# initc3/HoneyBadgerMPC

Hardware: AMD Instinct MI355X
Metric: shares reconstructed/sec (batch open, n=64 t=21) (higher is better)
Workload: dtype u256 (integer mod p): exact int8 x int8 -> int32 byte-split GEMM on the matrix cores; the high half of every sum folded mod p on the matrix cores too, one-word Barrett quotient

## Files before the change

### honeybadgermpc_amd/csrc/hb_common.hpp

```cpp
#pragma once
#include <hip/hip_runtime.h>
#include <stdint.h>
#include <stdio.h>
#include <string.h>

#include <functional>
#include <map>
#include <mutex>
#include <string>
#include <vector>

#include "../../include/hbmpc_hip.h"
#include "fp29.hpp"

namespace hb {
struct FastMatrix;
struct Mm8Matrix;
struct Mm8wMatrix;
}
namespace hb {

struct Wide { static constexpr int NL = 9, NW = 8; };
struct Narrow { static constexpr int NL = 3, NW = 2; };

// ... 14 lines not shown
        load_digits<NL, NW>(cd, poly + (size_t)l * NW);
        mont_mul(m, cd, pw, P);
        fp_add(acc, acc, m, P);
    }
#pragma unroll
    for (int q = 0; q < NL; q++) red[tid][q] = acc[q];
    __syncthreads();
    for (int w = 64; w >= 1; w >>= 1) {
        if (tid < w) {
            uint32_t a[NL], b[NL], t[NL];
#pragma unroll
            for (int q = 0; q < NL; q++) { a[q] = red[tid][q]; b[q] = red[tid + w][q]; }
            fp_add(t, a, b, P);
#pragma unroll
            for (int q = 0; q < NL; q++) red[tid][q] = t[q];
        }
        __syncthreads();
    }
#pragma unroll
    for (int q = 0; q < NL; q++) r[q] = red[0][q];
}

__host__ __device__ inline size_t m_index(int i, int l, int n_in, int nl, int q) {
    return (((size_t)((i / OT) * n_in + l) * (size_t)nl + (size_t)q) * OT) + (size_t)(i % OT);
}
inline int m_tiles(int n_out) { return (n_out + OT - 1) / OT; }

}

struct hb_matrix {
    hb_ctx *ctx;
    int n_out, n_in;
    uint32_t *dev;
    size_t words;
    bool cached;
    int refs;
    hb::Mm8wMatrix *wide;
    bool wide_tried;
};

namespace hb {
struct TlsError {
    static std::string &slot() { static thread_local std::string s; return s; }
    TlsError &operator=(const std::string &m) { slot() = m; return *this; }
    TlsError &operator=(const char *m) { slot() = m ? m : ""; return *this; }
    const char *c_str() const { return slot().c_str(); }
    void clear() { slot().clear(); }
    bool empty() const { return slot().empty(); }
};
struct PrescaleParams {
    uint32_t pbar[9];
    uint32_t pneg[8];
    uint32_t m0, m1;
};
}
namespace hb {
enum EnvHook {
    ENV_CACHE_CAP,
    ENV_GAO_PAIR,
    ENV_MM8W_FLAT,
    ENV_MM8W_RQ,
    ENV_MM8W_TILE16,
    ENV_MM8_NO_SKIP,
    ENV_NO_EVAL_FEW,
    ENV_NO_FUSED_SMALL,
    ENV_NO_FUSED_VALIDATE,
    ENV_NO_MFMA,
    ENV_NO_MFMA_DECODE,
    ENV_NO_MFMA_WIDE,
    ENV_NO_NARROW_FAST,
    ENV_NO_QUICK,
    ENV_NO_QUICK_PLAN,
    ENV_NTT_STAGE_LOOP,
    ENV_PROBE_WGS,
    ENV_QUICK_NO_CAND,
    ENV_UPLOAD_MODE,
    ENV_WB_NO_GAO,
    ENV_WB_NO_UNIFORM,
    ENV_COUNT
};
const char *env_hook(EnvHook h);
void env_reload();
}
struct hb_ctx {
    int device;
    int n_limbs;
    hb::FpParams<9> pw;
    hb::FpParams<3> pn;
    uint64_t p_limbs[4];
    std::recursive_mutex mu;
    int api_depth = 0;
    hb::TlsError err;
    std::map<std::string, hb_matrix *> mcache;
    std::map<std::vector<int32_t>, int32_t *> icache;
    std::map<std::string, void *> dcache;
    std::map<std::string, hb::FastMatrix *> fcache;
    std::map<std::string, hb::Mm8Matrix *> m8cache;
    struct CacheSlot { uint64_t tick; bool pinned; std::function<void()> drop; };
    std::map<std::string, CacheSlot> lru;
    uint64_t lru_clock = 0;
    size_t cache_cap = 192;
    int32_t *flag_dev;
    hb::PrescaleParams psc;
    int psc_state = 0;
    std::map<std::string, void *> ptcache;
    struct QuickSlot { void *buf = nullptr; size_t cap = 0; void *ev = nullptr; };
// ... 234 lines not shown
```

### honeybadgermpc_amd/csrc/hb_mfma.hip

```cpp
#include <atomic>

#include "hb_mm8.hpp"

namespace hb {

#include "hb_mm8_body.inc"

#ifdef HB_MM8_TIMING
__device__ unsigned long long g_mm8_t[2048 * 8];
#define MM8_T(k) do { const unsigned long long tn_ = __builtin_amdgcn_s_memtime(); tacc[k] += tn_ - tlast; tlast = tn_; } while (0)
#else
#define MM8_T(k) do { } while (0)
#endif
template <int NKB, bool CHECK, bool RAGGED, bool SKIP>
__global__ __launch_bounds__(256, 2) void k_mm8(const int4 *__restrict__ a8, const uint32_t *__restrict__ crowd,
                                                const uint32_t *__restrict__ zero_src,
                                                const uint32_t *__restrict__ in_pk, int64_t in_sc, int64_t in_sl,
                                                const int32_t *__restrict__ in_rows, int64_t in_count, int d,
                                                uint32_t *__restrict__ out_pk, int64_t out_sc, int64_t out_sl, int64_t out_count,
                                                const int32_t *__restrict__ check_mask, const int32_t *__restrict__ check_rows, int32_t *__restrict__ mismatch,
                                                uint32_t *__restrict__ copy_dst, int64_t copy_sc, int64_t copy_sl, int64_t copy_count, int copy_rows,
                                                int n_out, int n_rt, int tpw, int64_t n_chunks, int64_t n_units, BarrettParams bp) {
    extern __shared__ uint4 mm8_lds[];
    const int lane = threadIdx.x & 63, wave = __builtin_amdgcn_readfirstlane(threadIdx.x >> 6);
// ... 311 lines not shown
    uint64_t cy = 0;
    for (size_t i = 0; i < a.size(); i++) {
        uint64_t t = (uint64_t)a[i] + (i < b.size() ? b[i] : 0) + cy;
        a[i] = (uint32_t)t; cy = t >> 32;
    }
}
Big big_divmod(const Big &x, const Big &p, Big *q) {
    Big r(p.size() + 1, 0), pp(p); pp.push_back(0);
    if (q) q->assign(x.size(), 0);
    for (int bit = (int)x.size() * 32 - 1; bit >= 0; bit--) {
        uint32_t in = (x[bit >> 5] >> (bit & 31)) & 1u;
        for (size_t i = r.size(); i-- > 0;) r[i] = (r[i] << 1) | (i ? r[i - 1] >> 31 : in);
        if (big_ge(r, pp)) { big_sub(r, pp); if (q) (*q)[bit >> 5] |= 1u << (bit & 31); }
    }
    r.pop_back();
    return r;
}
Big big_shl(const Big &a, int bits, size_t words) {
    Big r(words, 0);
    for (size_t i = 0; i < a.size(); i++) {
        const size_t w = i + bits / 32; const int s = bits % 32;
        if (w < words) r[w] |= a[i] << s;
        if (s && w + 1 < words) r[w + 1] |= a[i] >> (32 - s);
    }
    return r;
}

}

namespace hb {

bool prescale_params(hb_ctx *ctx) {
    if (ctx->psc_state) return ctx->psc_state > 0;
    ctx->psc_state = -1;
    if (ctx->n_limbs != 4 || (ctx->p_limbs[3] >> 62) == 0) return false;
    Big p(8);
    for (int i = 0; i < 4; i++) { p[2 * i] = (uint32_t)ctx->p_limbs[i]; p[2 * i + 1] = (uint32_t)(ctx->p_limbs[i] >> 32); }
    Big pw9(p); pw9.push_back(0);
    Big pb(9, 0); pb[8] = 1u << 5;
    big_sub(pb, pw9);
    for (int k = 0; k < 9; k++) {
        const int bit = 29 * k, j = bit >> 5, sft = bit & 31;
        const uint64_t v = pb[j] | ((uint64_t)(j + 1 < 9 ? pb[j + 1] : 0) << 32);
        ctx->psc.pbar[k] = (uint32_t)(v >> sft) & DMASK;
    }
    Big pn(9, 0); pn[8] = 1;
    big_sub(pn, pw9);
    for (int k = 0; k < 8; k++) ctx->psc.pneg[k] = pn[k];
    Big two290(10, 0); two290[9] = 1u << 2;
    Big mu; big_divmod(two290, p, &mu);
    const uint64_t muv = mu[0] | ((uint64_t)mu[1] << 32);
    ctx->psc.m0 = (uint32_t)muv & DMASK;
    ctx->psc.m1 = (uint32_t)(muv >> LB);
    ctx->psc_state = 1;
    return true;
}

void mm8_free(Mm8Matrix *m) {
    if (!m) return;
    (void)hipFree(m->a8); (void)hipFree(m->crow); (void)hipFree(m->zero);
    delete m;
}

int mm8_shared(hb_ctx *ctx, const Mm8Shared **out, hipStream_t s) {
    if (ctx->mm8_shared) { *out = static_cast<const Mm8Shared *>(ctx->mm8_shared); return HB_OK; }
    if (ctx->n_limbs != 4 || (ctx->p_limbs[3] >> 62) == 0 || !prescale_params(ctx)) return fail(ctx, HB_ERR_UNSUPPORTED, "mm8: modulus");
    Mm8Shared *sh = new Mm8Shared();
    memset(sh, 0, sizeof *sh);
    Big p(8);
    for (int k = 0; k < 4; k++) { p[2 * k] = (uint32_t)ctx->p_limbs[k]; p[2 * k + 1] = (uint32_t)(ctx->p_limbs[k] >> 32); }
    uint32_t shift8[8];
    if (!fold_tables(ctx, 16, sh->fold_host, sh->bp.c384, &sh->bp.mu, shift8)) { delete sh; return fail(ctx, HB_ERR_UNSUPPORTED, "mm8: fold table"); }
    {
        Big pn(9, 0); pn[8] = 1;
        Big pw9(p); pw9.push_back(0);
        big_sub(pn, pw9);
        for (int k = 0; k < 8; k++) sh->bp.pneg[k] = pn[k];
    }
    auto digits9 = [](const Big &v, uint32_t *dg) {
        for (int k = 0; k < 9; k++) {
            const int bit = 29 * k, j = bit >> 5, sft = bit & 31;
            const uint64_t w = (uint64_t)(j < (int)v.size() ? v[j] : 0) | ((uint64_t)(j + 1 < (int)v.size() ? v[j + 1] : 0) << 32);
            dg[k] = (uint32_t)(w >> sft) & DMASK;
        }
    };
    Big biasmod;
    { Big bt(14, 0); for (int c = 0; c < MM8_NC; c++) { Big t(1, (uint32_t)MM8_BIAS); big_add(bt, big_shl(t, 8 * c, 14)); } biasmod = big_divmod(bt, p, nullptr); }
    { Big sft(shift8, shift8 + 8); if (!big_ge(biasmod, sft)) big_add(biasmod, p); big_sub(biasmod, sft); }
    digits9(biasmod, sh->biasmod);
    {
        Big c80(8, 0x80808080u);
        Big r261(9, 0); r261[8] = 1u << 5;
        digits9(big_divmod(big_mul(c80, r261), p, nullptr), sh->c80r);
    }
    if (hipMalloc(&sh->fold_dev, sizeof sh->fold_host) != hipSuccess) { delete sh; return fail(ctx, HB_ERR_HIP, "mm8: hipMalloc(fold table)"); }
    if (int rc = upload_table(ctx, sh->fold_dev, sh->fold_host, sizeof sh->fold_host, s)) { (void)hipFree(sh->fold_dev); delete sh; return rc; }
    ctx->mm8_shared = sh;
    *out = sh;
    return HB_OK;
}

void mm8_shared_free(hb_ctx *ctx) {
    Mm8Shared *sh = static_cast<Mm8Shared *>(ctx->mm8_shared);
    if (!sh) return;
    (void)hipFree(sh->fold_dev);
    delete sh;
// ... 171 lines not shown
```

### honeybadgermpc_amd/csrc/hb_mfma_fused.hip

```cpp
#include <math.h>

#include <algorithm>
#include <atomic>

#include "hb_mm8.hpp"

namespace hb {

#include "hb_mm8_body.inc"

constexpr int FS_WAVES = 8, FS_TPW = 4;
#ifdef HB_MM8_TIMING
__device__ unsigned long long g_fs_t[256 * 8 * 8];
#define FS_T(k) do { const unsigned long long tn_ = __builtin_amdgcn_s_memtime(); tacc[k] += tn_ - tlast; tlast = tn_; } while (0)
#else
#define FS_T(k) do { } while (0)
#endif
constexpr int FS_MAXD = 24, FS_MAXC = 104;
constexpr size_t FS_LDS_LIMIT = 156 * 1024;

struct FsIdx { uint16_t z[FS_MAXD], xz[FS_MAXD], zc[FS_MAXC], xzc[FS_MAXC]; };
struct FsPick { const uint4 *cand; const uint32_t *cand_crow; int n_coef, nc; uint16_t zc[FS_MAXC]; };
struct FsSplit { uint32_t terms[FS_WAVES]; };
constexpr int FS_CAND_MAXN = 128;

__host__ __device__ inline size_t fs_lds_bytes(int n_rt, int nkb) {
    return ((size_t)n_rt * 64 + (size_t)n_rt * nkb * 2 * 64 + (size_t)2 * FS_TPW * nkb * 4 * 64 + MM8_FOLD_Q) * 16 + (size_t)(32 + 16 * n_rt) * 4;
}

template <int NKB>
__global__ __launch_bounds__(64 * FS_WAVES, 2) void k_mm8f(const int4 *__restrict__ a8, const uint32_t *__restrict__ crowd, const v4i *__restrict__ foldg,
                                                          const uint32_t *__restrict__ KT, const PrescaleParams PP,
                                                          const uint32_t *__restrict__ in_pk, int64_t in_sc, int64_t in_sl, const int32_t *__restrict__ in_rows,
                                                          int64_t in_count, int d, const int32_t *__restrict__ rowmode,
                                                          uint32_t *__restrict__ out_pk, int64_t out_sc, int64_t out_sl, int64_t out_count,
                                                          int32_t *__restrict__ mismatch, int32_t *__restrict__ first_bad, uint32_t *__restrict__ bad_map,
                                                          int n_out, int n_rt, int64_t n_chunks, int64_t n_units, BarrettParams bp, const FsDone done, const FsPick pick,
                                                          const FsSplit split) {
    constexpr int NT = 64 * FS_WAVES, NL = 9, NW = 8;
    extern __shared__ uint4 fs_lds[];
    const int lane = threadIdx.x & 63, wave = __builtin_amdgcn_readfirstlane(threadIdx.x >> 6);
    const int n = lane & 15, g = lane >> 4;
    uint32_t *crl = reinterpret_cast<uint32_t *>(fs_lds);
    int4 *abuf = reinterpret_cast<int4 *>(fs_lds + n_rt * 64);
    uint4 *xbuf = fs_lds + n_rt * 64 + n_rt * NKB * 2 * 64;
    constexpr int bufsz = FS_TPW * NKB * 4 * 64;
    int32_t *rowl = reinterpret_cast<int32_t *>(xbuf + 2 * bufsz);
    int32_t *maskl = rowl + 32;
    v4i *foldl = reinterpret_cast<v4i *>(maskl + 16 * n_rt);

    if (threadIdx.x < 32) {
        const int lc = (int)threadIdx.x < d ? (int)threadIdx.x : d - 1;
        rowl[threadIdx.x] = in_rows ? in_rows[lc] : lc;
    }
    uint4 pk_piece = make_uint4(0, 0, 0, 0), pk_crow = make_uint4(0, 0, 0, 0);
    const int pk_e = threadIdx.x;
    const bool pk_has_piece = pick.cand && pk_e < pick.nc * NKB * 8, pk_has_crow = pick.cand && pk_e < pick.nc * 4;
    if (pk_has_piece) {
        const int j = pk_e / (NKB * 8), pc = pk_e - j * (NKB * 8);
        pk_piece = pick.cand[(size_t)pick.zc[j] * (NKB * 8) + pc];
    }
    if (pk_has_crow) pk_crow = reinterpret_cast<const uint4 *>(pick.cand_crow)[(size_t)pick.zc[pk_e >> 2] * 4 + (pk_e & 3)];
    for (int i = threadIdx.x; i < n_rt * 16; i += NT) maskl[i] = i < n_out ? rowmode[i] : 0;
    for (int i = threadIdx.x; i < n_rt * 64; i += NT) fs_lds[i] = reinterpret_cast<const uint4 *>(crowd)[i];
    for (int i = threadIdx.x; i < n_rt * NKB * 2 * 64; i += NT) abuf[i] = a8[i];
    for (int i = threadIdx.x; i < 2 * bufsz; i += NT) xbuf[i] = make_uint4(0, 0, 0, 0);
    if (threadIdx.x < MM8_FOLD_Q) foldl[threadIdx.x] = foldg[threadIdx.x];
    if (pick.cand) {
        __syncthreads();
        auto put = [&](int e, const uint4 &v) {
            const int j = e / (NKB * 8), pc = e - j * (NKB * 8);
            const int ri = pick.n_coef + j, rt = ri >> 4, r16 = ri & 15, r = 4 * (r16 & 3) + (r16 >> 2);
            const int kb = pc >> 3, grp = (pc >> 2) & 1, gg = pc & 3;
            reinterpret_cast<uint4 *>(abuf)[((rt * NKB + kb) * 2 + grp) * 64 + r + 16 * gg] = v;
        };
        if (pk_has_piece) put(pk_e, pk_piece);
        for (int e = pk_e + NT; e < pick.nc * NKB * 8; e += NT) {
            const int j = e / (NKB * 8), pc = e - j * (NKB * 8);
            put(e, pick.cand[(size_t)pick.zc[j] * (NKB * 8) + pc]);
        }
        if (pk_has_crow) fs_lds[(pick.n_coef + (pk_e >> 2)) * 4 + (pk_e & 3)] = pk_crow;
        for (int j = threadIdx.x; j < pick.nc; j += NT) maskl[pick.n_coef + j] = (int32_t)pick.zc[j] + 1;
    }
    __syncthreads();

    const int n_pairs = FS_TPW * n_rt;
    const uint32_t my_terms = (uint32_t)__builtin_amdgcn_readfirstlane((int)split.terms[wave]);

    auto scale_unit = [&](int64_t unit, uint4 *dst, uint32_t terms) {
        int64_t chunk = unit * 64 + lane;
        if (chunk >= n_chunks) chunk = n_chunks - 1;
        const int t = lane >> 4;
        uint32_t xw[NW];
        bool ok = false;
        auto fetch = [&](int l, uint32_t (&w)[NW], bool &okk) {
            const int64_t idx = chunk * in_sc + (int64_t)rowl[l] * in_sl;
            okk = idx < in_count;
            load_words<NW>(w, in_pk + (okk ? idx : 0) * NW);
        };
        terms &= d < 32 ? (1u << d) - 1u : ~0u;
        int l = terms ? __builtin_ctz(terms) : d;
        if (l < d) fetch(l, xw, ok);
        while (l < d) {
            terms &= terms - 1u;
            const int ln = terms ? __builtin_ctz(terms) : d;
            uint32_t xn[NW];
            bool okn = false;
            if (ln < d) fetch(ln, xn, okn);
            else {
#pragma unroll
                for (int k = 0; k < NW; k++) xn[k] = 0;
            }
            const uint32_t *__restrict__ T = KT + (size_t)l * (NL * NL);
            uint32_t xd[NL];
            unpack<NL, NW>(xd, xw);
            uint64_t col[NL + 1];
#pragma unroll
            for (int j = 0; j <= NL; j++) col[j] = 0;
#pragma unroll
            for (int q = 0; q < NL; q++)
#pragma unroll
                for (int j = 0; j < NL; j++) col[j] += (uint64_t)xd[q] * T[q * NL + j];
            uint32_t v[NL + 1];
#pragma unroll
            for (int k = 0; k < NL; k++) { v[k] = (uint32_t)col[k] & DMASK; col[k + 1] += col[k] >> LB; }
            v[NL] = (uint32_t)col[NL];
            const uint64_t mid = (uint64_t)v[9] * PP.m0 + (uint64_t)v[8] * PP.m1 + (((uint64_t)v[8] * PP.m0) >> LB);
            const uint64_t qh = (uint64_t)v[9] * PP.m1 + (mid >> LB);
            const uint32_t q0 = (uint32_t)qh & DMASK, q1 = (uint32_t)(qh >> LB);
            uint64_t dc[NL];
#pragma unroll
            for (int k = 0; k < NL; k++) {
                dc[k] = v[k] + (uint64_t)q0 * PP.pbar[k];
                if (k > 0) dc[k] += (uint64_t)q1 * PP.pbar[k - 1];
            }
            uint32_t r[NL];
#pragma unroll
            for (int k = 0; k < NL; k++) {
                r[k] = (uint32_t)dc[k] & DMASK;
                if (k < NL - 1) dc[k + 1] += dc[k] >> LB;
            }
            uint32_t w[NW];
            pack<NL, NW>(w, r);
            if (PP.pneg[NW - 1] >> 31) {
#pragma unroll
                for (int k = 0; k < NW; k++) w[k] = ok ? w[k] : 0u;
            } else {
                uint32_t u[NW];
                unsigned cy = 0;
#pragma unroll
                for (int k = 0; k < NW; k++) u[k] = __builtin_addc(w[k], PP.pneg[k], cy, &cy);
                const bool take = cy || (r[NL - 1] >> 24);
#pragma unroll
                for (int k = 0; k < NW; k++) w[k] = ok ? (take ? u[k] : w[k]) : 0u;
            }
            const int kb = l >> 3, gg = (l & 7) >> 1, e = l & 1;
            uint4 *slot = dst + (size_t)(((t * NKB + kb) * 2 + e) * 2) * 64 + (n + 16 * gg);
            slot[0] = make_uint4(w[0], w[1], w[2], w[3]);
            slot[64] = make_uint4(w[4], w[5], w[6], w[7]);
#pragma unroll
            for (int k = 0; k < NW; k++) xw[k] = xn[k];
            ok = okn;
            l = ln;
        }
    };

    const v4i biasv = v4i{MM8_BIAS, MM8_BIAS, MM8_BIAS, MM8_BIAS};
    uint32_t k256 = 256u, k16m = 1u << 24;
    int32_t s1 = 1, s256 = 256, s64k = 1 << 16, s16m = 1 << 24;
    uint32_t u1 = 1u;
    asm volatile("" : "+s"(k256), "+s"(k16m), "+s"(s1), "+s"(s256), "+s"(s64k), "+s"(s16m), "+s"(u1));
    const v4i *fold_lane = reinterpret_cast<const v4i *>(reinterpret_cast<const char *>(foldl) + (g == (n >> 2) ? 16 * n : 256));

    int buf = 0;
    int64_t unit = blockIdx.x;
#ifdef HB_MM8_TIMING
    unsigned long long tacc[8] = {0, 0, 0, 0, 0, 0, 0, 0}, tlast = __builtin_amdgcn_s_memtime();
#endif
    if (unit < n_units) scale_unit(unit, xbuf, 0x01010101u << wave);
    FS_T(0);
    for (; unit < n_units; unit += gridDim.x, buf ^= 1) {
        asm volatile("s_waitcnt lgkmcnt(0)" ::: "memory");
        FS_T(7);
        __builtin_amdgcn_s_barrier();
        FS_T(1);
        if (my_terms && unit + gridDim.x < n_units) scale_unit(unit + gridDim.x, xbuf + (size_t)(buf ^ 1) * bufsz, my_terms);
        FS_T(2);
        for (int pidx = wave; pidx < n_pairs; pidx += FS_WAVES) {
            const int tl = n_rt == 2 ? (pidx >> 1) : pidx / n_rt;
            const int rt = n_rt == 2 ? ((pidx ^ (pidx >> 2)) & 1) : pidx - tl * n_rt;
            const int64_t chunk = (unit * FS_TPW + tl) * 16 + n;
            const uint4 *xs = xbuf + (size_t)buf * bufsz + (size_t)tl * NKB * 4 * 64 + lane;
            const int4 *as = abuf + (size_t)rt * NKB * 2 * 64 + lane;
            uint32_t eap[4][11], c0p[4];
            const int rows_here = n_out - 16 * rt < 16 ? n_out - 16 * rt : 16;
            const int nreg = (rows_here + 3) >> 2;
            const uint32_t xs_addr = (uint32_t)(uintptr_t)(__attribute__((address_space(3))) const void *)xs;
            const uint32_t as_addr = (uint32_t)(uintptr_t)(__attribute__((address_space(3))) const void *)as;
            {
                v4i acc[24];
                asm volatile("" ::: "memory");
                __builtin_amdgcn_sched_barrier(0);
                __builtin_amdgcn_s_setprio(0);
                Mm8Phase<NKB, 0, false>::run(acc, xs_addr, as_addr, biasv);
                __builtin_amdgcn_s_setprio(2);
                __builtin_amdgcn_sched_barrier(0);
                FS_T(3);
#pragma unroll
                for (int reg = 0; reg < 4; reg++) {
                    if (reg >= 2 && reg >= nreg) break;
                    c0p[reg] = (uint32_t)acc[0][reg];
#pragma unroll
                    for (int j = 0; j < 11; j++) eap[reg][j] = (uint32_t)acc[1 + 2 * j][reg] + ((uint32_t)acc[2 + 2 * j][reg] << 8);
                    asm volatile("" ::"v"(c0p[reg]), "v"(eap[reg][0]), "v"(eap[reg][1]), "v"(eap[reg][2]), "v"(eap[reg][3]), "v"(eap[reg][4]),
                                 "v"(eap[reg][5]), "v"(eap[reg][6]), "v"(eap[reg][7]), "v"(eap[reg][8]), "v"(eap[reg][9]), "v"(eap[reg][10]));
                    __builtin_amdgcn_sched_barrier(0);
// ... 108 lines not shown
            FS_T(6);
        }
    }
#ifdef HB_MM8_TIMING
    if (lane == 0 && blockIdx.x < 256) for (int k = 0; k < 8; k++) g_fs_t[(blockIdx.x * 8 + wave) * 8 + k] = tacc[k];
#endif
    fs_workgroup_done(done, mismatch, first_bad);
}

typedef __int128 i128;

struct FsConsts { uint32_t c80r[9], biasmod[9]; };
constexpr int32_t FS_OVERFLOW = 0x40000000;

__device__ __forceinline__ size_t fs_digit_addr(int i, int l, int b, int nkb) {
    const int lane_ = (4 * ((i % 16) % 4) + (i % 16) / 4) + 16 * ((l % 8) / 2), el = l & 1;
    const int grp = b >> 3, r7 = 7 - (b & 7), hi = r7 >> 2, bi = r7 & 3;
    return ((((size_t)(i / 16) * nkb + l / 8) * 2 + grp) * 64 + (size_t)lane_) * 16 + 4 * (2 * hi + el) + bi;
}

__device__ __forceinline__ void fs_row_constant(const FpParams<9> &P, const FsConsts &cs, const i128 *row, int d, uint32_t *dst16) {
    constexpr int NL = 9, NW = 8;
    uint32_t s5[5] = {0, 0, 0, 0, 0};
    for (int l = 0; l < d; l++) {
        const i128 v = row[l];
        const uint32_t vw[5] = {(uint32_t)v, (uint32_t)(v >> 32), (uint32_t)(v >> 64), (uint32_t)(v >> 96), (uint32_t)(v >> 127 >> 1)};
        unsigned cy = 0;
#pragma unroll
        for (int k = 0; k < 5; k++) s5[k] = __builtin_addc(s5[k], vw[k], cy, &cy);
    }
    const bool negs = (s5[4] >> 31) != 0;
    if (negs) {
        unsigned cy = 1;
#pragma unroll
        for (int k = 0; k < 5; k++) s5[k] = __builtin_addc(~s5[k], 0u, cy, &cy);
    }
    uint32_t w8[NW] = {s5[0], s5[1], s5[2], s5[3], s5[4], 0, 0, 0}, fe[NL], prod[NL], corr[NL], k80[NL], bm[NL];
    unpack<NL, NW>(fe, w8);
    if (negs) fp_neg(fe, fe, P);
#pragma unroll
    for (int k = 0; k < NL; k++) { k80[k] = cs.c80r[k]; bm[k] = cs.biasmod[k]; }
    mont_mul(prod, fe, k80, P);
    fp_sub(corr, prod, bm, P);
    uint32_t cw[NW];
    pack<NL, NW>(cw, corr);
#pragma unroll
    for (int k = 0; k < 8; k++) {
        const uint64_t pair = (uint64_t)cw[k] + ((0x1010ull << 32) | 0x10100000ull);
        dst16[2 * k] = (uint32_t)pair;
        dst16[2 * k + 1] = (uint32_t)(pair >> 32);
    }
}

__device__ __forceinline__ void fs_build_body(uint8_t *fb_lds, const FpParams<9> &P, const uint32_t *__restrict__ inv, int n, const FsIdx &ix, int d, int nc, int n_coef,
                                              int flags, const FsConsts &cs, uint8_t *__restrict__ a8, uint32_t *__restrict__ crow, uint32_t *__restrict__ KT,
                                              int32_t *__restrict__ rowmode, int32_t *__restrict__ z_dev, int32_t *__restrict__ status) {
    constexpr int NL = 9, NW = 8;
    const int n_out = n_coef + nc, nkb = (d + 7) / 8, n_rt = (n_out + 15) / 16;
    i128 *ent = reinterpret_cast<i128 *>(fb_lds);
    i128 *Ac = ent + (size_t)n_out * d;
    uint32_t *wj = reinterpret_cast<uint32_t *>(Ac + (d + 1));
    uint32_t *part = wj + (size_t)d * NL;
    const int tid = threadIdx.x;
    const bool do_z = flags & FS_BUILD_Z, do_zc = flags & FS_BUILD_ZC;
    if (do_z) {
        const size_t img = (size_t)n_rt * nkb * 2 * 64 * 16;
        for (size_t i = tid; i < img / 16; i += 1024) reinterpret_cast<uint4 *>(a8)[i] = make_uint4(0, 0, 0, 0);
        for (int i = tid; i < n_rt * 16 * 8; i += 1024) { crow[2 * i] = 0x10100000u; crow[2 * i + 1] = 0x1010u; }
        for (int i = tid; i < n_rt * 16; i += 1024) rowmode[i] = i < n_coef ? -(i + 1) : 0;
        if (tid < d) z_dev[tid] = ix.z[tid];
    }
    if (do_z && tid < 64) {
        if (tid <= d) Ac[tid] = tid == 0 ? 1 : 0;
        __builtin_amdgcn_fence(__ATOMIC_RELEASE, "wavefront");
        __builtin_amdgcn_wave_barrier();
        for (int q = 0; q < d; q++) {
            i128 nv = 0;
            const bool act = tid <= q + 1 && tid <= d;
            if (act) nv = (tid > 0 ? Ac[tid - 1] : (i128)0) - (i128)ix.xz[q] * Ac[tid];
            __builtin_amdgcn_fence(__ATOMIC_ACQ_REL, "wavefront");
            __builtin_amdgcn_wave_barrier();
            if (act) Ac[tid] = nv;
            __builtin_amdgcn_fence(__ATOMIC_ACQ_REL, "wavefront");
            __builtin_amdgcn_wave_barrier();
        }
        if (tid < d) {
            const i128 xj = ix.xz[tid];
            i128 cur = 1;
            for (int m = d - 1; m >= 0; m--) {
                if (m < n_coef) ent[(size_t)m * d + tid] = cur;
                if (m > 0) cur = Ac[m] + xj * cur;
            }
        }
    } else if (do_z && tid < 64 + 4 * FS_MAXD + 32) {
        const int j = (tid - 64) >> 2, pq = (tid - 64) & 3;
        if (j < d) {
            uint32_t w[NL];
            fp_set(w, P.one);
            const uint32_t *row = inv + (size_t)ix.z[j] * n * NL;
            for (int q = pq; q < d; q += 4) {
                if (q == j) continue;
                uint32_t f[NL];
#pragma unroll
                for (int k = 0; k < NL; k++) f[k] = row[(size_t)ix.z[q] * NL + k];
                mont_mul(w, w, f, P);
            }
#pragma unroll
            for (int k = 0; k < NL; k++) part[((size_t)j * 4 + pq) * NL + k] = w[k];
        }
    } else if (do_zc && tid >= 256) {
        for (int e = tid - 256; e < nc * d; e += 1024 - 256) {
            const int i = e / d, j = e - i * d;
            const int64_t xi = ix.xzc[i];
            i128 v = 1;
            for (int q = 0; q < d; q++)
                if (q != j) v *= (i128)(xi - (int64_t)ix.xz[q]);
            ent[(size_t)(n_coef + i) * d + j] = v;
        }
    }
    __syncthreads();
    if (do_z && tid < d) {
        uint32_t a[NL], b[NL], c[NL];
#pragma unroll
        for (int k = 0; k < NL; k++) { a[k] = part[((size_t)tid * 4) * NL + k]; b[k] = part[((size_t)tid * 4 + 1) * NL + k]; }
        mont_mul(c, a, b, P);
#pragma unroll
        for (int k = 0; k < NL; k++) { a[k] = part[((size_t)tid * 4 + 2) * NL + k]; b[k] = part[((size_t)tid * 4 + 3) * NL + k]; }
        mont_mul(a, a, b, P);
        mont_mul(c, c, a, P);
#pragma unroll
        for (int k = 0; k < NL; k++) wj[(size_t)tid * NL + k] = c[k];
    }
    __syncthreads();
    const int row_lo = do_z ? 0 : n_coef, row_hi = do_zc ? n_out : n_coef;
    for (int e = tid + row_lo * d; e < row_hi * d; e += 1024) {
        const int i = e / d, l = e - i * d;
        i128 v = ent[e];
        const bool negv = v < 0;
        int carry = 0;
#pragma unroll
        for (int b = 0; b < 16; b++) {
            int t = (int)((uint32_t)(v >> (8 * b)) & 0xffu) + carry;
            if (t > 127) { t -= 256; carry = 1; } else carry = 0;
            a8[fs_digit_addr(i, l, b, nkb)] = (uint8_t)(int8_t)t;
        }
        if (carry != (negv ? 1 : 0) && status) atomicOr(status, FS_OVERFLOW);
    }
    for (int i = tid + row_lo; i < row_hi; i += 1024) fs_row_constant(P, cs, ent + (size_t)i * d, d, crow + (size_t)i * 16);
    if (do_zc)
        for (int i = tid; i < nc; i += 1024) rowmode[n_coef + i] = (int32_t)ix.zc[i] + 1;
    if (do_z) {
        for (int e = tid; e < d * NL; e += 1024) {
            const int l = e / NL, q = e - l * NL;
            uint32_t w[NL], two[NL], tq[NL];
#pragma unroll
            for (int k = 0; k < NL; k++) { w[k] = wj[(size_t)l * NL + k]; two[k] = (k == q) ? 1u : 0u; }
            mont_mul(tq, w, two, P);
#pragma unroll
            for (int k = 0; k < NL; k++) KT[((size_t)l * NL + q) * NL + k] = tq[k];
        }
    }
}

__device__ __forceinline__ void fs_cand_body(uint8_t *fc_lds, const FpParams<9> &P, int n, const uint16_t *__restrict__ xs, const FsIdx &ix, int d, const FsConsts &cs,
                                             uint8_t *__restrict__ cand, uint32_t *__restrict__ cand_crow, int32_t *__restrict__ status) {
    i128 *ent = reinterpret_cast<i128 *>(fc_lds);
    const int tid = threadIdx.x, nkb = (d + 7) / 8;
    const size_t row_bytes = (size_t)nkb * 8 * 16;
    for (size_t i = tid; i < (size_t)n * row_bytes / 16; i += 1024) reinterpret_cast<uint4 *>(cand)[i] = make_uint4(0, 0, 0, 0);
    for (int e = tid; e < n * d; e += 1024) {
        const int i = e / d, j = e - i * d;
        const int64_t xi = xs[i];
        i128 v = 1;
        for (int q = 0; q < d; q++)
            if (q != j) v *= (i128)(xi - (int64_t)ix.xz[q]);
        ent[e] = v;
    }
    __syncthreads();
    for (int e = tid; e < n * d; e += 1024) {
        const int i = e / d, l = e - i * d;
        const i128 v = ent[e];
        const bool negv = v < 0;
        const int kb = l >> 3, gg = (l & 7) >> 1, el = l & 1;
        int carry = 0;
#pragma unroll
        for (int b = 0; b < 16; b++) {
            int t = (int)((uint32_t)(v >> (8 * b)) & 0xffu) + carry;
            if (t > 127) { t -= 256; carry = 1; } else carry = 0;
            const int grp = b >> 3, r7 = 7 - (b & 7), hi = r7 >> 2, bi = r7 & 3;
            cand[(size_t)i * row_bytes + (size_t)(((kb * 2 + grp) * 4 + gg) * 16) + 4 * (2 * hi + el) + bi] = (uint8_t)(int8_t)t;
        }
        if (carry != (negv ? 1 : 0) && status) atomicOr(status, FS_OVERFLOW);
    }
    for (int i = tid; i < n; i += 1024) fs_row_constant(P, cs, ent + (size_t)i * d, d, cand_crow + (size_t)i * 16);
}

__global__ void __launch_bounds__(1024) k_fs_build(const FpParams<9> P, const uint32_t *__restrict__ inv, int n, const FsIdx ix, int d, int nc, int n_coef,
                                                   int flags, const FsConsts cs, uint8_t *__restrict__ a8, uint32_t *__restrict__ crow, uint32_t *__restrict__ KT,
                                                   int32_t *__restrict__ rowmode, int32_t *__restrict__ z_dev, int32_t *__restrict__ status) {
    extern __shared__ __attribute__((aligned(16))) uint8_t fs_b_lds[];
    fs_build_body(fs_b_lds, P, inv, n, ix, d, nc, n_coef, flags, cs, a8, crow, KT, rowmode, z_dev, status);
}

__global__ void __launch_bounds__(1024) k_fs_cand(const FpParams<9> P, int n, const uint16_t *__restrict__ xs, const FsIdx ix, int d, const FsConsts cs,
                                                  uint8_t *__restrict__ cand, uint32_t *__restrict__ cand_crow, int32_t *__restrict__ status) {
    extern __shared__ __attribute__((aligned(16))) uint8_t fs_c_lds[];
    fs_cand_body(fs_c_lds, P, n, xs, ix, d, cs, cand, cand_crow, status);
}

__global__ void __launch_bounds__(1024) k_fs_build_z_cand(const FpParams<9> P, const uint32_t *__restrict__ inv, int n, const uint16_t *__restrict__ xs, const FsIdx ix, int d, int nc,
                                                          int n_coef, const FsConsts cs, uint8_t *__restrict__ a8, uint32_t *__restrict__ crow, uint32_t *__restrict__ KT,
                                                          int32_t *__restrict__ rowmode, int32_t *__restrict__ z_dev, uint8_t *__restrict__ cand, uint32_t *__restrict__ cand_crow,
                                                          int32_t *__restrict__ status) {
    extern __shared__ __attribute__((aligned(16))) uint8_t fs_zc_lds[];
    if (blockIdx.x == 0) fs_build_body(fs_zc_lds, P, inv, n, ix, d, nc, n_coef, FS_BUILD_Z, cs, a8, crow, KT, rowmode, z_dev, status);
    else fs_cand_body(fs_zc_lds, P, n, xs, ix, d, cs, cand, cand_crow, status);
}

static int fs_num_cus() {
    static int n = 0;
    if (!n) {
        int dev = 0;
        (void)hipGetDevice(&dev);
        if (hipDeviceGetAttribute(&n, hipDeviceAttributeMultiprocessorCount, dev) != hipSuccess || n <= 0) n = 256;
    }
    return n;
}

int fs_layout(hb_ctx *ctx, const PointTable *pt, int d, int nc, int n_coef, FsLayout *L) {
    if (ctx->n_limbs != 4 || !pt || !pt->usable || !pt->small) return HB_ERR_UNSUPPORTED;
    if (d < 4 || d > 22 || nc < 0 || nc > FS_MAXC || n_coef < 1 || n_coef > d) return HB_ERR_UNSUPPORTED;
    if (env_hook(ENV_NO_MFMA) || env_hook(ENV_NO_FUSED_SMALL) || env_hook(ENV_NO_QUICK) || !prescale_params(ctx)) return HB_ERR_UNSUPPORTED;
    if ((int64_t)d * 16 * 128 * 128 > MM8_BIAS) return HB_ERR_UNSUPPORTED;
    std::vector<uint16_t> xs(pt->xs);
    std::sort(xs.begin(), xs.end());
    double bits_n = 0.0, bits_p = 0.0;
    for (int k = 0; k < d - 1 && k < (int)xs.size(); k++) bits_n += log2(1.0 + xs[xs.size() - 1 - k]);
    const int R = xs.empty() ? 0 : xs.back() - xs.front();
    for (int k = 0; k < d - 1; k++) { const int dist = R - k / 2; if (dist < 1) break; bits_p += log2((double)dist); }
    if (bits_n > 124.5 || bits_p > 124.5) return HB_ERR_UNSUPPORTED;
    L->n = pt->n; L->d = d; L->nc = nc; L->n_coef = n_coef; L->n_out = n_coef + nc;
    L->nkb = (d + 7) / 8; L->n_rt = (L->n_out + 15) / 16;
    if (fs_lds_bytes(L->n_rt, L->nkb) > FS_LDS_LIMIT) return HB_ERR_UNSUPPORTED;
    auto al = [](size_t v) { return (v + 255) & ~(size_t)255; };
    L->o_a8 = 0;
    L->o_crow = al((size_t)L->n_rt * L->nkb * 2 * 64 * 16);
    L->o_kt = L->o_crow + al((size_t)L->n_rt * 16 * 16 * 4);
    L->o_mode = L->o_kt + al((size_t)d * 81 * 4);
    L->o_z = L->o_mode + al((size_t)L->n_rt * 16 * 4);
    L->need = L->o_z + al((size_t)FS_MAXD * 4);
    L->o_cand = L->o_cand_crow = 0;
    if (pt->n <= FS_CAND_MAXN && nc > 0) {
        L->o_cand = L->need;
        L->o_cand_crow = L->o_cand + al((size_t)pt->n * L->nkb * 8 * 16);
        L->need = L->o_cand_crow + al((size_t)pt->n * 16 * 4);
    }
    return HB_OK;
}

int fs_build(hb_ctx *ctx, const PointTable *pt, const int32_t *z, const int32_t *zc, const FsLayout &L, uint8_t *base, int flags, int32_t *status_dev, hipStream_t s) {
    const int n = L.n, d = L.d, nc = L.nc;
    FsIdx ix;
    memset(&ix, 0, sizeof ix);
    uint64_t seen[4] = {0, 0, 0, 0};
    std::vector<uint8_t> seen_big;
    if (n > 256) seen_big.assign((size_t)n, 0);
    auto mark = [&](int v) -> bool {
        if (v < 0 || v >= n) return false;
        if (n > 256) { if (seen_big[v]) return false; seen_big[v] = 1; return true; }
        if (seen[v >> 6] >> (v & 63) & 1) return false;
        seen[v >> 6] |= 1ull << (v & 63);
        return true;
    };
    for (int i = 0; i < d; i++) { if (!mark(z[i])) return fail(ctx, HB_ERR_BAD_ARG, "fused decode: arrival indices"); ix.z[i] = (uint16_t)z[i]; ix.xz[i] = pt->xs[z[i]]; }
    if (flags & FS_BUILD_ZC)
        for (int j = 0; j < nc; j++) { if (!mark(zc[j])) return fail(ctx, HB_ERR_BAD_ARG, "fused decode: compared indices"); ix.zc[j] = (uint16_t)zc[j]; ix.xzc[j] = pt->xs[zc[j]]; }
    const Mm8Shared *sh = nullptr;
    int rc = mm8_shared(ctx, &sh, s); if (rc) return rc;
    FsConsts cs;
    memcpy(cs.c80r, sh->c80r, sizeof cs.c80r);
    memcpy(cs.biasmod, sh->biasmod, sizeof cs.biasmod);
    const size_t lds = ((size_t)L.n_out * d + d + 1) * 16 + ((size_t)d * 9 + (size_t)d * 4 * 9) * 4;
    k_fs_build<<<1, 1024, lds, s>>>(ctx->pw, pt->inv, n, ix, d, nc, L.n_coef, flags, cs, base + L.o_a8, (uint32_t *)(base + L.o_crow), (uint32_t *)(base + L.o_kt),
                                    (int32_t *)(base + L.o_mode), (int32_t *)(base + L.o_z), status_dev);
    HB_LAUNCH_CHECK(ctx);
    return HB_OK;
}

int fs_build_cand(hb_ctx *ctx, PointTable *pt, const int32_t *z, const FsLayout &L, uint8_t *base, int32_t *status_dev, hipStream_t s, bool with_z) {
    if (!L.o_cand) return fail(ctx, HB_ERR_BAD_ARG, "fused decode: no candidate store in this layout");
    if (!pt->xs_dev) {
        HB_HIP(ctx, hipMalloc(&pt->xs_dev, (size_t)pt->n * 2));
        int rc = upload_table(ctx, pt->xs_dev, pt->xs.data(), (size_t)pt->n * 2, s);
        if (rc) { (void)hipFree(pt->xs_dev); pt->xs_dev = nullptr; return rc; }
    }
    FsIdx ix;
    memset(&ix, 0, sizeof ix);
    uint64_t seen[2] = {0, 0};
    for (int i = 0; i < L.d; i++) {
        const int v = z[i];
        if (v < 0 || v >= pt->n || (seen[v >> 6] >> (v & 63) & 1)) return fail(ctx, HB_ERR_BAD_ARG, "fused decode: arrival indices");
        seen[v >> 6] |= 1ull << (v & 63);
        ix.z[i] = (uint16_t)v; ix.xz[i] = pt->xs[v];
    }
    const Mm8Shared *sh = nullptr;
    int rc = mm8_shared(ctx, &sh, s); if (rc) return rc;
    FsConsts cs;
    memcpy(cs.c80r, sh->c80r, sizeof cs.c80r);
    memcpy(cs.biasmod, sh->biasmod, sizeof cs.biasmod);
    if (with_z) {
        const size_t lds_b = ((size_t)L.n_out * L.d + L.d + 1) * 16 + ((size_t)L.d * 9 + (size_t)L.d * 4 * 9) * 4, lds_c = (size_t)pt->n * L.d * 16;
        k_fs_build_z_cand<<<2, 1024, std::max(lds_b, lds_c), s>>>(ctx->pw, pt->inv, pt->n, pt->xs_dev, ix, L.d, L.nc, L.n_coef, cs, base + L.o_a8, (uint32_t *)(base + L.o_crow),
                                                                  (uint32_t *)(base + L.o_kt), (int32_t *)(base + L.o_mode), (int32_t *)(base + L.o_z), base + L.o_cand,
                                                                  (uint32_t *)(base + L.o_cand_crow), status_dev);
        HB_LAUNCH_CHECK(ctx);
        return HB_OK;
    }
    k_fs_cand<<<1, 1024, (size_t)pt->n * L.d * 16, s>>>(ctx->pw, pt->n, pt->xs_dev, ix, L.d, cs, base + L.o_cand, (uint32_t *)(base + L.o_cand_crow), status_dev);
    HB_LAUNCH_CHECK(ctx);
    return HB_OK;
}

static FsSplit fs_split(int d, int n_rt, int n_out) {
    constexpr int PASS = 95, RAGGED = 70, TERM = 36;
    FsSplit sp;
    int load[FS_WAVES];
    const int n_pairs = FS_TPW * n_rt;
    const bool ragged = n_out - 16 * (n_rt - 1) <= 8;
    for (int w = 0; w < FS_WAVES; w++) {
        sp.terms[w] = 0;
        load[w] = 0;
        for (int pidx = w; pidx < n_pairs; pidx += FS_WAVES) {
            const int tl = n_rt == 2 ? (pidx >> 1) : pidx / n_rt;
            const int rt = n_rt == 2 ? ((pidx ^ (pidx >> 2)) & 1) : pidx - tl * n_rt;
            load[w] += (ragged && rt == n_rt - 1) ? RAGGED : PASS;
        }
    }
    for (int l = 0; l < d; l++) {
        int best = FS_WAVES - 1;
        for (int w = FS_WAVES - 2; w >= 0; w--)
            if (load[w] < load[best]) best = w;
        sp.terms[best] |= 1u << l;
        load[best] += TERM;
    }
    return sp;
}

int fs_launch(hb_ctx *ctx, const FsLayout &L, const uint8_t *base, const uint32_t *cols, hb_view cv, uint32_t *out, hb_view ov, int64_t out_count,
              int32_t *mismatch_dev, int32_t *first_bad_dev, uint32_t *bad_map_dev, int64_t C, hipStream_t s, const FsDone *done_p, const int32_t *pick_zc) {
    FsDone done;
    memset(&done, 0, sizeof done);
    if (done_p) done = *done_p;
    FsPick pick;
    memset(&pick, 0, sizeof pick);
    if (pick_zc) {
        if (!L.o_cand) return fail(ctx, HB_ERR_BAD_ARG, "fused decode: no candidate store to pick from");
        pick.cand = (const uint4 *)(base + L.o_cand); pick.cand_crow = (const uint32_t *)(base + L.o_cand_crow);
        pick.n_coef = L.n_coef; pick.nc = L.nc;
        for (int j = 0; j < L.nc; j++) pick.zc[j] = (uint16_t)pick_zc[j];
    }
    if (C <= 0) return HB_OK;
    const Mm8Shared *sh = nullptr;
    int rc = mm8_shared(ctx, &sh, s); if (rc) return rc;
    const int64_t n_units = (C + 63) / 64;
    int64_t blocks = fs_num_cus();
    if (blocks > n_units) blocks = n_units;
    blocks = mm8_trimmed_grid(n_units, blocks);
    const size_t lds = fs_lds_bytes(L.n_rt, L.nkb);
    const FsSplit split = fs_split(L.d, L.n_rt, L.n_out);
#define FS_LAUNCH(NKB)                                                                                                                     \
    do {                                                                                                                                   \
        static std::atomic<unsigned long long> attr_done{0};                                                                                                        \
        if (!((attr_done.load() >> (ctx->device & 63)) & 1ull)) { HB_HIP(ctx, hipFuncSetAttribute(reinterpret_cast<const void *>(k_mm8f<NKB>), hipFuncAttributeMaxDynamicSharedMemorySize, 160 * 1024)); attr_done.fetch_or(1ull << (ctx->device & 63)); } \
        k_mm8f<NKB><<<dim3((unsigned)blocks), dim3(64 * FS_WAVES), lds, s>>>((const int4 *)(base + L.o_a8), (const uint32_t *)(base + L.o_crow), sh->fold_dev,        \
            (const uint32_t *)(base + L.o_kt), ctx->psc, cols, cv.stride_c, cv.stride_l, (const int32_t *)(base + L.o_z), INT64_MAX, L.d, (const int32_t *)(base + L.o_mode), \
            out, ov.stride_c, ov.stride_l, out_count, mismatch_dev, first_bad_dev, bad_map_dev, L.n_out, L.n_rt, C, n_units, sh->bp, done, pick, split); \
    } while (0)
    switch (L.nkb) {
        case 1: FS_LAUNCH(1); break;
        case 2: FS_LAUNCH(2); break;
        case 3: FS_LAUNCH(3); break;
        default: return fail(ctx, HB_ERR_UNSUPPORTED, "fused decode: more than 24 terms");
    }
#undef FS_LAUNCH
    HB_LAUNCH_CHECK(ctx);
    return HB_OK;
}

}

#ifdef HB_MM8_TIMING
extern "C" int hb_debug_fs_timing(unsigned long long *out, int count) {
    return hipMemcpyFromSymbol(out, HIP_SYMBOL(hb::g_fs_t), sizeof(unsigned long long) * (size_t)count) == hipSuccess ? 0 : 1;
}
#endif
```

Measured before the change: 8.366 billion.

## Prescale fused-decode terms directly on packed words with per-term constant table

Rebuilds the per-term prescale table so it multiplies the 8 packed 32-bit input words directly, removing the unpack to 29-bit limbs and the final pack step. The Barrett quotient now uses a rescaled mu (2^292/p), and the reduction constants are stored in each term's table row so they load from memory rather than from kernel arguments. Input fetches use a wave-uniform row offset without bounds checks and are double-buffered across two terms. The per-term load-balance cost constant is lowered to match the cheaper term, which changes how terms are assigned to waves. The dropped bounds check assumes all rows are in range.

```diff
diff --git a/honeybadgermpc_amd/csrc/hb_common.hpp b/honeybadgermpc_amd/csrc/hb_common.hpp
--- a/honeybadgermpc_amd/csrc/hb_common.hpp
+++ b/honeybadgermpc_amd/csrc/hb_common.hpp
@@ -90,6 +90,7 @@
     uint32_t pbar[9];
     uint32_t pneg[8];
     uint32_t m0, m1;
+    uint32_t u0, u1;
 };
 }
 namespace hb {
diff --git a/honeybadgermpc_amd/csrc/hb_mfma.hip b/honeybadgermpc_amd/csrc/hb_mfma.hip
--- a/honeybadgermpc_amd/csrc/hb_mfma.hip
+++ b/honeybadgermpc_amd/csrc/hb_mfma.hip
@@ -387,6 +387,11 @@
     const uint64_t muv = mu[0] | ((uint64_t)mu[1] << 32);
     ctx->psc.m0 = (uint32_t)muv & DMASK;
     ctx->psc.m1 = (uint32_t)(muv >> LB);
+    Big two292(10, 0); two292[9] = 1u << 4;
+    Big mu2; big_divmod(two292, p, &mu2);
+    const uint64_t mu2v = mu2[0] | ((uint64_t)mu2[1] << 32);
+    ctx->psc.u0 = (uint32_t)mu2v & DMASK;
+    ctx->psc.u1 = (uint32_t)(mu2v >> LB);
     ctx->psc_state = 1;
     return true;
 }
diff --git a/honeybadgermpc_amd/csrc/hb_mfma_fused.hip b/honeybadgermpc_amd/csrc/hb_mfma_fused.hip
--- a/honeybadgermpc_amd/csrc/hb_mfma_fused.hip
+++ b/honeybadgermpc_amd/csrc/hb_mfma_fused.hip
@@ -17,6 +17,7 @@
 #define FS_T(k) do { } while (0)
 #endif
 constexpr int FS_MAXD = 24, FS_MAXC = 104;
+constexpr int FS_KT_PBAR = 72, FS_KT_MU = 81, FS_KT_PNEG = 88, FS_KT_WORDS = 96;
 constexpr size_t FS_LDS_LIMIT = 156 * 1024;
 
 struct FsIdx { uint16_t z[FS_MAXD], xz[FS_MAXD], zc[FS_MAXC], xzc[FS_MAXC]; };
@@ -30,9 +31,9 @@
 
 template <int NKB>
 __global__ __launch_bounds__(64 * FS_WAVES, 2) void k_mm8f(const int4 *__restrict__ a8, const uint32_t *__restrict__ crowd, const v4i *__restrict__ foldg,
-                                                          const uint32_t *__restrict__ KT, const PrescaleParams PP,
+                                                          const uint32_t *__restrict__ KT,
                                                           const uint32_t *__restrict__ in_pk, int64_t in_sc, int64_t in_sl, const int32_t *__restrict__ in_rows,
-                                                          int64_t in_count, int d, const int32_t *__restrict__ rowmode,
+                                                          int d, const int32_t *__restrict__ rowmode,
                                                           uint32_t *__restrict__ out_pk, int64_t out_sc, int64_t out_sl, int64_t out_count,
                                                           int32_t *__restrict__ mismatch, int32_t *__restrict__ first_bad, uint32_t *__restrict__ bad_map,
                                                           int n_out, int n_rt, int64_t n_chunks, int64_t n_units, BarrettParams bp, const FsDone done, const FsPick pick,
@@ -91,77 +92,73 @@
         int64_t chunk = unit * 64 + lane;
         if (chunk >= n_chunks) chunk = n_chunks - 1;
         const int t = lane >> 4;
-        uint32_t xw[NW];
-        bool ok = false;
-        auto fetch = [&](int l, uint32_t (&w)[NW], bool &okk) {
-            const int64_t idx = chunk * in_sc + (int64_t)rowl[l] * in_sl;
-            okk = idx < in_count;
-            load_words<NW>(w, in_pk + (okk ? idx : 0) * NW);
+        const uint32_t *__restrict__ xin = in_pk + chunk * in_sc * NW;
+        auto fetch = [&](int l, uint32_t (&w)[NW]) {
+            const int64_t roff = (int64_t)__builtin_amdgcn_readfirstlane(rowl[l]) * in_sl * NW;
+            load_words<NW>(w, xin + roff);
         };
-        terms &= d < 32 ? (1u << d) - 1u : ~0u;
-        int l = terms ? __builtin_ctz(terms) : d;
-        if (l < d) fetch(l, xw, ok);
-        while (l < d) {
-            terms &= terms - 1u;
-            const int ln = terms ? __builtin_ctz(terms) : d;
-            uint32_t xn[NW];
-            bool okn = false;
-            if (ln < d) fetch(ln, xn, okn);
-            else {
-#pragma unroll
-                for (int k = 0; k < NW; k++) xn[k] = 0;
+        auto term = [&](int l, const uint32_t (&xw)[NW]) {
+            const uint32_t *__restrict__ T = KT + (size_t)l * FS_KT_WORDS;
+            const uint32_t *__restrict__ pbar = T + FS_KT_PBAR, *__restrict__ pneg = T + FS_KT_PNEG;
+            uint32_t v[NL + 1];
+            uint64_t acc = 0;
+#pragma unroll
+            for (int k = 0; k < NL; k++) {
+#pragma unroll
+                for (int j = 0; j < NW; j++) acc += (uint64_t)xw[j] * T[k * NW + j];
+                v[k] = (uint32_t)acc & DMASK;
+                acc >>= LB;
             }
-            const uint32_t *__restrict__ T = KT + (size_t)l * (NL * NL);
-            uint32_t xd[NL];
-            unpack<NL, NW>(xd, xw);
-            uint64_t col[NL + 1];
-#pragma unroll
-            for (int j = 0; j <= NL; j++) col[j] = 0;
-#pragma unroll
-            for (int q = 0; q < NL; q++)
-#pragma unroll
-                for (int j = 0; j < NL; j++) col[j] += (uint64_t)xd[q] * T[q * NL + j];
-            uint32_t v[NL + 1];
-#pragma unroll
-            for (int k = 0; k < NL; k++) { v[k] = (uint32_t)col[k] & DMASK; col[k + 1] += col[k] >> LB; }
-            v[NL] = (uint32_t)col[NL];
-            const uint64_t mid = (uint64_t)v[9] * PP.m0 + (uint64_t)v[8] * PP.m1 + (((uint64_t)v[8] * PP.m0) >> LB);
-            const uint64_t qh = (uint64_t)v[9] * PP.m1 + (mid >> LB);
-            const uint32_t q0 = (uint32_t)qh & DMASK, q1 = (uint32_t)(qh >> LB);
-            uint64_t dc[NL];
+            v[NL] = (uint32_t)acc;
+            const uint32_t mu0 = T[FS_KT_MU], mu1 = T[FS_KT_MU + 1];
+            const uint64_t mid = (uint64_t)v[9] * mu0 + (uint64_t)v[8] * mu1;
+            const uint64_t qh = (uint64_t)v[9] * mu1 + (mid >> LB);
+            const uint32_t q0 = (uint32_t)(qh >> 2) & DMASK, q1 = (uint32_t)(qh >> (LB + 2));
+            uint32_t a[NL];
+            acc = 0;
 #pragma unroll
             for (int k = 0; k < NL; k++) {
-                dc[k] = v[k] + (uint64_t)q0 * PP.pbar[k];
-                if (k > 0) dc[k] += (uint64_t)q1 * PP.pbar[k - 1];
-            }
-            uint32_t r[NL];
-#pragma unroll
-            for (int k = 0; k < NL; k++) {
-                r[k] = (uint32_t)dc[k] & DMASK;
-                if (k < NL - 1) dc[k + 1] += dc[k] >> LB;
+                acc += v[k];
+                acc += (uint64_t)q0 * pbar[k];
+                if (k > 0) acc += (uint64_t)q1 * pbar[k - 1];
+                a[k] = (uint32_t)acc;
+                acc >>= LB;
             }
             uint32_t w[NW];
-            pack<NL, NW>(w, r);
-            if (PP.pneg[NW - 1] >> 31) {
-#pragma unroll
-                for (int k = 0; k < NW; k++) w[k] = ok ? w[k] : 0u;
-            } else {
+#pragma unroll
+            for (int j = 0; j < NW; j++) {
+                const int i = 32 * j / LB, o = 32 * j % LB;
+                w[j] = ((a[i] & DMASK) >> o) | (a[i + 1] << (LB - o));
+            }
+            if (!(pneg[NW - 1] >> 31)) {
                 uint32_t u[NW];
                 unsigned cy = 0;
 #pragma unroll
-                for (int k = 0; k < NW; k++) u[k] = __builtin_addc(w[k], PP.pneg[k], cy, &cy);
-                const bool take = cy || (r[NL - 1] >> 24);
-#pragma unroll
-                for (int k = 0; k < NW; k++) w[k] = ok ? (take ? u[k] : w[k]) : 0u;
+                for (int k = 0; k < NW; k++) u[k] = __builtin_addc(w[k], pneg[k], cy, &cy);
+                const bool take = cy || ((a[NL - 1] & DMASK) >> 24);
+#pragma unroll
+                for (int k = 0; k < NW; k++) w[k] = take ? u[k] : w[k];
             }
             const int kb = l >> 3, gg = (l & 7) >> 1, e = l & 1;
             uint4 *slot = dst + (size_t)(((t * NKB + kb) * 2 + e) * 2) * 64 + (n + 16 * gg);
             slot[0] = make_uint4(w[0], w[1], w[2], w[3]);
             slot[64] = make_uint4(w[4], w[5], w[6], w[7]);
-#pragma unroll
-            for (int k = 0; k < NW; k++) xw[k] = xn[k];
-            ok = okn;
-            l = ln;
+        };
+        terms &= d < 32 ? (1u << d) - 1u : ~0u;
+        int l = terms ? __builtin_ctz(terms) : d;
+        uint32_t xa[NW], xb[NW];
+        if (l < d) fetch(l, xa);
+        while (l < d) {
+            terms &= terms - 1u;
+            const int l2 = terms ? __builtin_ctz(terms) : d;
+            fetch(l2 < d ? l2 : l, xb);
+            term(l, xa);
+            if (l2 >= d) break;
+            terms &= terms - 1u;
+            const int l3 = terms ? __builtin_ctz(terms) : d;
+            fetch(l3 < d ? l3 : l2, xa);
+            term(l2, xb);
+            l = l3;
         }
     };
 
@@ -376,7 +373,7 @@
     }
 }
 
-__device__ __forceinline__ void fs_build_body(uint8_t *fb_lds, const FpParams<9> &P, const uint32_t *__restrict__ inv, int n, const FsIdx &ix, int d, int nc, int n_coef,
+__device__ __forceinline__ void fs_build_body(uint8_t *fb_lds, const FpParams<9> &P, const PrescaleParams &PP, const uint32_t *__restrict__ inv, int n, const FsIdx &ix, int d, int nc, int n_coef,
                                               int flags, const FsConsts &cs, uint8_t *__restrict__ a8, uint32_t *__restrict__ crow, uint32_t *__restrict__ KT,
                                               int32_t *__restrict__ rowmode, int32_t *__restrict__ z_dev, int32_t *__restrict__ status) {
     constexpr int NL = 9, NW = 8;
@@ -474,14 +471,19 @@
     if (do_zc)
         for (int i = tid; i < nc; i += 1024) rowmode[n_coef + i] = (int32_t)ix.zc[i] + 1;
     if (do_z) {
-        for (int e = tid; e < d * NL; e += 1024) {
-            const int l = e / NL, q = e - l * NL;
+        for (int e = tid; e < d * NW; e += 1024) {
+            const int l = e / NW, q = e - l * NW;
             uint32_t w[NL], two[NL], tq[NL];
 #pragma unroll
-            for (int k = 0; k < NL; k++) { w[k] = wj[(size_t)l * NL + k]; two[k] = (k == q) ? 1u : 0u; }
+            for (int k = 0; k < NL; k++) { w[k] = wj[(size_t)l * NL + k]; two[k] = (k == 32 * q / LB) ? 1u << (32 * q % LB) : 0u; }
             mont_mul(tq, w, two, P);
 #pragma unroll
-            for (int k = 0; k < NL; k++) KT[((size_t)l * NL + q) * NL + k] = tq[k];
+            for (int k = 0; k < NL; k++) KT[(size_t)l * FS_KT_WORDS + k * NW + q] = tq[k];
+        }
+        for (int e = tid; e < d * (FS_KT_WORDS - FS_KT_PBAR); e += 1024) {
+            const int l = e / (FS_KT_WORDS - FS_KT_PBAR), i = FS_KT_PBAR + e % (FS_KT_WORDS - FS_KT_PBAR);
+            const uint32_t c = i < FS_KT_MU ? PP.pbar[i - FS_KT_PBAR] : i == FS_KT_MU ? PP.u0 : i == FS_KT_MU + 1 ? PP.u1 : i >= FS_KT_PNEG ? PP.pneg[i - FS_KT_PNEG] : 0u;
+            KT[(size_t)l * FS_KT_WORDS + i] = c;
         }
     }
 }
@@ -519,11 +521,11 @@
     for (int i = tid; i < n; i += 1024) fs_row_constant(P, cs, ent + (size_t)i * d, d, cand_crow + (size_t)i * 16);
 }
 
-__global__ void __launch_bounds__(1024) k_fs_build(const FpParams<9> P, const uint32_t *__restrict__ inv, int n, const FsIdx ix, int d, int nc, int n_coef,
+__global__ void __launch_bounds__(1024) k_fs_build(const FpParams<9> P, const PrescaleParams PP, const uint32_t *__restrict__ inv, int n, const FsIdx ix, int d, int nc, int n_coef,
                                                    int flags, const FsConsts cs, uint8_t *__restrict__ a8, uint32_t *__restrict__ crow, uint32_t *__restrict__ KT,
                                                    int32_t *__restrict__ rowmode, int32_t *__restrict__ z_dev, int32_t *__restrict__ status) {
     extern __shared__ __attribute__((aligned(16))) uint8_t fs_b_lds[];
-    fs_build_body(fs_b_lds, P, inv, n, ix, d, nc, n_coef, flags, cs, a8, crow, KT, rowmode, z_dev, status);
+    fs_build_body(fs_b_lds, P, PP, inv, n, ix, d, nc, n_coef, flags, cs, a8, crow, KT, rowmode, z_dev, status);
 }
 
 __global__ void __launch_bounds__(1024) k_fs_cand(const FpParams<9> P, int n, const uint16_t *__restrict__ xs, const FsIdx ix, int d, const FsConsts cs,
@@ -532,12 +534,12 @@
     fs_cand_body(fs_c_lds, P, n, xs, ix, d, cs, cand, cand_crow, status);
 }
 
-__global__ void __launch_bounds__(1024) k_fs_build_z_cand(const FpParams<9> P, const uint32_t *__restrict__ inv, int n, const uint16_t *__restrict__ xs, const FsIdx ix, int d, int nc,
+__global__ void __launch_bounds__(1024) k_fs_build_z_cand(const FpParams<9> P, const PrescaleParams PP, const uint32_t *__restrict__ inv, int n, const uint16_t *__restrict__ xs, const FsIdx ix, int d, int nc,
                                                           int n_coef, const FsConsts cs, uint8_t *__restrict__ a8, uint32_t *__restrict__ crow, uint32_t *__restrict__ KT,
                                                           int32_t *__restrict__ rowmode, int32_t *__restrict__ z_dev, uint8_t *__restrict__ cand, uint32_t *__restrict__ cand_crow,
                                                           int32_t *__restrict__ status) {
     extern __shared__ __attribute__((aligned(16))) uint8_t fs_zc_lds[];
-    if (blockIdx.x == 0) fs_build_body(fs_zc_lds, P, inv, n, ix, d, nc, n_coef, FS_BUILD_Z, cs, a8, crow, KT, rowmode, z_dev, status);
+    if (blockIdx.x == 0) fs_build_body(fs_zc_lds, P, PP, inv, n, ix, d, nc, n_coef, FS_BUILD_Z, cs, a8, crow, KT, rowmode, z_dev, status);
     else fs_cand_body(fs_zc_lds, P, n, xs, ix, d, cs, cand, cand_crow, status);
 }
 
@@ -570,7 +572,7 @@
     L->o_a8 = 0;
     L->o_crow = al((size_t)L->n_rt * L->nkb * 2 * 64 * 16);
     L->o_kt = L->o_crow + al((size_t)L->n_rt * 16 * 16 * 4);
-    L->o_mode = L->o_kt + al((size_t)d * 81 * 4);
+    L->o_mode = L->o_kt + al((size_t)d * FS_KT_WORDS * 4);
     L->o_z = L->o_mode + al((size_t)L->n_rt * 16 * 4);
     L->need = L->o_z + al((size_t)FS_MAXD * 4);
     L->o_cand = L->o_cand_crow = 0;
@@ -605,7 +607,7 @@
     memcpy(cs.c80r, sh->c80r, sizeof cs.c80r);
     memcpy(cs.biasmod, sh->biasmod, sizeof cs.biasmod);
     const size_t lds = ((size_t)L.n_out * d + d + 1) * 16 + ((size_t)d * 9 + (size_t)d * 4 * 9) * 4;
-    k_fs_build<<<1, 1024, lds, s>>>(ctx->pw, pt->inv, n, ix, d, nc, L.n_coef, flags, cs, base + L.o_a8, (uint32_t *)(base + L.o_crow), (uint32_t *)(base + L.o_kt),
+    k_fs_build<<<1, 1024, lds, s>>>(ctx->pw, ctx->psc, pt->inv, n, ix, d, nc, L.n_coef, flags, cs, base + L.o_a8, (uint32_t *)(base + L.o_crow), (uint32_t *)(base + L.o_kt),
                                     (int32_t *)(base + L.o_mode), (int32_t *)(base + L.o_z), status_dev);
     HB_LAUNCH_CHECK(ctx);
     return HB_OK;
@@ -634,7 +636,7 @@
     memcpy(cs.biasmod, sh->biasmod, sizeof cs.biasmod);
     if (with_z) {
         const size_t lds_b = ((size_t)L.n_out * L.d + L.d + 1) * 16 + ((size_t)L.d * 9 + (size_t)L.d * 4 * 9) * 4, lds_c = (size_t)pt->n * L.d * 16;
-        k_fs_build_z_cand<<<2, 1024, std::max(lds_b, lds_c), s>>>(ctx->pw, pt->inv, pt->n, pt->xs_dev, ix, L.d, L.nc, L.n_coef, cs, base + L.o_a8, (uint32_t *)(base + L.o_crow),
+        k_fs_build_z_cand<<<2, 1024, std::max(lds_b, lds_c), s>>>(ctx->pw, ctx->psc, pt->inv, pt->n, pt->xs_dev, ix, L.d, L.nc, L.n_coef, cs, base + L.o_a8, (uint32_t *)(base + L.o_crow),
                                                                   (uint32_t *)(base + L.o_kt), (int32_t *)(base + L.o_mode), (int32_t *)(base + L.o_z), base + L.o_cand,
                                                                   (uint32_t *)(base + L.o_cand_crow), status_dev);
         HB_LAUNCH_CHECK(ctx);
@@ -646,7 +648,7 @@
 }
 
 static FsSplit fs_split(int d, int n_rt, int n_out) {
-    constexpr int PASS = 95, RAGGED = 70, TERM = 36;
+    constexpr int PASS = 95, RAGGED = 70, TERM = 15;
     FsSplit sp;
     int load[FS_WAVES];
     const int n_pairs = FS_TPW * n_rt;
@@ -697,7 +699,7 @@
         static std::atomic<unsigned long long> attr_done{0};                                                                                                        \
         if (!((attr_done.load() >> (ctx->device & 63)) & 1ull)) { HB_HIP(ctx, hipFuncSetAttribute(reinterpret_cast<const void *>(k_mm8f<NKB>), hipFuncAttributeMaxDynamicSharedMemorySize, 160 * 1024)); attr_done.fetch_or(1ull << (ctx->device & 63)); } \
         k_mm8f<NKB><<<dim3((unsigned)blocks), dim3(64 * FS_WAVES), lds, s>>>((const int4 *)(base + L.o_a8), (const uint32_t *)(base + L.o_crow), sh->fold_dev,        \
-            (const uint32_t *)(base + L.o_kt), ctx->psc, cols, cv.stride_c, cv.stride_l, (const int32_t *)(base + L.o_z), INT64_MAX, L.d, (const int32_t *)(base + L.o_mode), \
+            (const uint32_t *)(base + L.o_kt), cols, cv.stride_c, cv.stride_l, (const int32_t *)(base + L.o_z), L.d, (const int32_t *)(base + L.o_mode), \
             out, ov.stride_c, ov.stride_l, out_count, mismatch_dev, first_bad_dev, bad_map_dev, L.n_out, L.n_rt, C, n_units, sh->bp, done, pick, split); \
     } while (0)
     switch (L.nkb) {
```

Result: faster. 8.741 billion (median of 6 runs) (+4.5%).
